# DTUWindEnergy/WindGym

Hardware: AMD Instinct MI355X
Metric: env-steps/sec (whole node), 16-turbine farm x 4096 envs (higher is better)
Workload: dtype f32

## Files before the change

### windgym_amd/csrc/wg_env.hip

```cpp
#include <hip/hip_runtime.h>

#ifndef WG_ENV_ABLATE
#define WG_ENV_ABLATE 0
#endif
#include "wg_env_common.h"
#include "wg_internal.h"

struct __attribute__((aligned(16))) EnvSlotLds {
    int dev_rem, fill_rem, sub, budget;
    double s_new;
    int n_emit, n_valid, new_valid;
    unsigned n_emitted;
    float s_off_f, near_f, move_max, ti_pow;
    double s_off, ws;
    float ws_f, ti_f, wd_env, base_acc;
    int n_pushed, pend_farm_n, pend_base_n, n_flow;
    double c_time;
    int c_head;
    unsigned c_part, c_flow, c_istep, c_tag, n_emitted0;
    float out_pw;
    unsigned c_add;
    int bg_init;
    int pad_[3];
};
// ... 133 lines not shown
            c_tag = (unsigned)cx.episode_tag; init_pending = cx.init_pending; time_max_c = cx.time_max;
            const int* ro = kl->d.roff + ctx_id * (unsigned)(N + 1);
            l_roff = ro[(unsigned)t]; l_rnext = ro[(unsigned)t + 1u];
            l_xr = kl->d.xr[tcx]; l_yr = kl->d.yr[tcx];
            l_yaw = kl->d.yaw[tb]; l_u = kl->d.u[tb]; l_ti = kl->d.ti_loc[tb];
            l_bnd = reinterpret_cast<const float4*>(kl->d.bnd)[tb];
        };
        load_state();
        const int n_tab = k0->p.n_tab, S = k0->p.S;
        const unsigned i_tab = (unsigned)min(tid, n_tab - 1), i_s = (unsigned)min(tid, S - 1);
        const float pf_tp = k0->d.tab_power[i_tab], pf_tc = k0->d.tab_ct[i_tab];
        const float pf_dy = k0->d.rotor_dy[i_s], pf_dz = k0->d.rotor_dz[i_s];
        {
            const bool has_act = mode == WG_MODE_STEP && farm == 0;
            const float a = *(has_act ? actions + (unsigned)(e * N + t) : k0->d.tab_ct);
            l_act = has_act ? a : 0.f;
        }

#define WG_HDR_I(f) __builtin_amdgcn_readlane(hw, (int)(offsetof(WgEnv, f) / 4))
        env_live = WG_HDR_I(live);
        int env_done = WG_HDR_I(done), env_shadow_iters = WG_HDR_I(shadow_iters), env_steps_done = WG_HDR_I(steps_done);
        int env_timestep = WG_HDR_I(timestep), env_time_max_live = WG_HDR_I(time_max_live);
#undef WG_HDR_I
        if (SPLIT && role == 1) {
            if (tid == 0) { *reinterpret_cast<int*>(smem + WG_ENV_OFF_HDR) = 0; if (GLUE != 0 && (SPLIT == 1 || wv == 0)) reinterpret_cast<int*>(zone)[LEAN_PRE_FLAG] = 0; }
            asm volatile("s_waitcnt vmcnt(0) lgkmcnt(0)" ::: "memory");
        }
        if (WPE == 2) {
            asm volatile("" : "+s"(env_live), "+s"(env_done), "+s"(env_shadow_iters), "+s"(env_steps_done), "+s"(env_timestep), "+s"(env_time_max_live) : : "memory");
            asm volatile("s_barrier" ::: "memory");
        }
        if (SPLIT && role == 1 && GLUE != 0 && c == env_live) {
            const EnvKArgsPtr kz = (EnvKArgsPtr)wg_cold_args();
            const WgParams& zp = *(const WgParams*)&kz->gp;
            const WgPtrs& zd = *(const WgPtrs*)&kz->gd;
#define WG_HDR_Z(f) __builtin_amdgcn_readlane(hw, (int)(offsetof(WgEnv, f) / 4))
            const int z_np = WG_HDR_Z(n_pushed_live), z_fn = WG_HDR_Z(farm_pow_n), z_bn = WG_HDR_Z(base_pow_n);
#undef WG_HDR_Z
            const int PA = zp.power_avg;
            const SumsRaw zr = wg_sums_load<false, false>(zp, zd, e, e * 2 + env_live, tid < N ? tid : 0, z_np);
            const float z_fo = zd.farm_pow[(size_t)e * PA + z_fn % PA];
            const float z_bo = F == 2 ? zd.base_pow[(size_t)e * PA + z_bn % PA] : 0.f;
            const float z_met = tid < WG_N_METRICS ? zd.metrics[(size_t)e * WG_N_METRICS + tid] : 0.f;
            double* const zs = reinterpret_cast<double*>(zone);
#pragma unroll
            for (int sI = 0; sI < WG_N_CH; ++sI) { zs[LEAN_PRE_S(sI, tid)] = zr.S[sI]; zone[LEAN_PRE_LV(sI, tid)] = zr.lv[sI]; }
            zone[LEAN_PRE_MET(tid)] = z_met;
            if (tid == 0) { zone[LEAN_PRE_FOLD] = z_fo; zone[LEAN_PRE_BOLD] = z_bo; }
            asm volatile("s_waitcnt lgkmcnt(0)" ::: "memory");
            if (tid == 0) env_flag_set(reinterpret_cast<int*>(zone) + LEAN_PRE_FLAG);
        }
        out.env_live = env_live;
        out.truncates = env_timestep >= env_time_max_live;
        out.steps_done = env_steps_done; out.time_max_live = env_time_max_live;

        const bool is_live_c = (c == env_live);
        const int autoreset = k0->p.autoreset;
        int budget = 0;
        long plan_left = 0;
        if (mode == WG_MODE_STEP) {
            role_live = is_live_c && !env_done;
            role_dev = !is_live_c && autoreset != 0;
            const int bg_pending = WPE == 2 ? (is_live_c ? 0 : __shfl(init_pending, 0, 64)) : __shfl(init_pending, (env_live ^ 1) * F * N, 64);
            out.bg_init_pending = autoreset && bg_pending;
            if (SPLIT == 2 && role == 1 && out.bg_init_pending) return;
            if (autoreset && bg_pending && WPE == 1 && !out.truncates) {
                defer_init = true;
                budget = 0;
            } else if (autoreset && bg_pending) {
                const KArgsPtr ki = wg_cold_args();
                const WgParams& gp = *ki->d.gp;
                env_init_episode<GLUE != 0>(e, env_live ^ 1, tid);
                full_barrier<64>();
                load_state();
                const int fill_max = F == 2 ? max(gp.fill_a, gp.fill_b) : gp.fill_a;
                const int inc = 1 + (gp.extra_inc ? 1 : 0);
                const int tm = WPE == 2 ? ki->d.ctx[e * 2 + env_live].time_max : __shfl(time_max_c, env_live * F * N, 64);
                const long total = (long)((tm + inc - 1) / inc) + 1;
                const int dev0 = __shfl(dev_rem, WPE == 2 ? 0 : (env_live ^ 1) * F * N, 64);
                budget = wg_shadow_share(dev0 + gp.K * fill_max, total - env_steps_done, env_steps_done, e);
                budget = wg_shadow_share(dev_rem + gp.K * fill_rem, total - env_steps_done, env_steps_done, e, farm ? 0x80000000u : 0u);
// ... 68 lines not shown
        float2* const rpt = reinterpret_cast<float2*>(tabct + n_tab);
        const float hub = k1->p.hub;
        auto rp = [&](const float dy_, const float dz_) __attribute__((always_inline)) {
            const float dz = hub + dz_ - hub;
            return make_float2(dy_, dz * dz);
        };
        if (tid < n_tab) { tabp[tid] = pf_tp; tabct[tid] = pf_tc; }
        if (tid < S) rpt[tid] = rp(pf_dy, pf_dz);
        for (int i = tid + 64; i < n_tab; i += 64) { tabp[i] = k1->d.tab_power[i]; tabct[i] = k1->d.tab_ct[i]; }
        for (int i = tid + 64; i < S; i += 64) rpt[i] = rp(k1->d.rotor_dy[i], k1->d.rotor_dz[i]);

        yaw = l_yaw; tu = l_u; tti = l_ti; oyaw = l_yaw;
        if (role_live && farm == 0 && valid) {
            const float a = l_act, ymin = k1->p.yaw_min, ymax = k1->p.yaw_max, ystep = k1->p.yaw_step;
            if (k1->p.action_method == WG_ACT_YAW) {
                yaw = fminf(fmaxf(yaw + a * ystep, ymin), ymax);
            } else {
                float tf = a + 1.0f;
                tf = tf * 0.5f;
                tf = tf * (ymax - ymin);
                tf = tf + ymin;
                const float ny = fminf(fmaxf(tf, yaw - ystep), yaw + ystep);
                yaw = fminf(fmaxf(ny, ymin), ymax);
            }
        }
    }
    float tpow = 0.f, tct = 0.f, cg = 1.f;
    float sws = 0.f, swd = 0.f, syaw = 0.f, sp_ = 0.f;
    int part_acc = 0, stream_acc = 0;
    bool stepped = false;
    lds_barrier<64>();
    WG_STAMP(1);

    for (int round = 0;; ++round) {
        bool stepping, is_dev;
        int sub, K;
        if (__ballot(parked)) {
            bool due = parked && SL[k - 1].dev_rem == 0;
            unsigned long long due_m = __ballot(due);
            if (due_m) {
                full_barrier<64>();
                const KArgsPtr kc = wg_cold_args();
                const unsigned pstride = (unsigned)kc->p.pstride;
                const size_t pb_env = (size_t)(e * 2 * F + kbase) * pstride;
                const int src_lane = (tid - N) & 63;
                const float c_tu = __shfl(tu, src_lane, 64), c_tti = __shfl(tti, src_lane, 64), c_pw = __shfl(tpow, src_lane, 64);
                const float c_ct = __shfl(tct, src_lane, 64), c_cg = __shfl(cg, src_lane, 64);
                if (due) { tu = c_tu; tti = c_tti; tpow = c_pw; tct = c_ct; cg = c_cg; stepped = true; parked = false; }
                while (due_m) {
                    const int kd = __builtin_amdgcn_readlane(k, __builtin_ctzll(due_m));
                    env_clone_dev(smem, kd, N, kc->p.P, kc->p.dt_d, kc->d.py + pb_env, kc->d.rec_a + 2 * pb_env, (unsigned)(kd - 1) * pstride,
                                  (unsigned)kd * pstride, tid);
                    due_m &= ~(((1ull << N) - 1ull) << (kd * N));
                }
                lds_barrier<64>();
            }
        }
        {
            const KArgsPtr kr = wg_cold_args();
            K = kr->p.K;
            const int4 sch = *reinterpret_cast<const int4*>(&my.dev_rem);
            const bool active = sch.x > 0 || sch.y > 0;
            stepping = valid && (role_live ? (round < K) : (role_dev && active && (sch.w > 0 || sch.z != 0)));
            is_dev = !role_live && sch.x > 0;
            sub = sch.z;
            if (!__ballot(stepping)) break;
        out.rounds = round + 1;
            if (round > 0) full_barrier<64>();

            if (role_live && farm == 1 && stepping) {
                const float ystep = kr->p.yaw_step;
                if (kr->p.base_controller == WG_CTRL_LOCAL) {
                    const float off = 0.f - yaw;
                    const float sgn = (float)((off > 0.f) - (off < 0.f));
                    yaw = yaw + sgn * fminf(fabsf(off), ystep);
                } else {
                    const float sgn = (float)((yaw > 0.f) - (yaw < 0.f));
                    yaw = yaw - sgn * fminf(fabsf(yaw), ystep);
                }
            }

            if (stepping && t == 0) {
                const double dpart = kr->p.dpart;
                const int P = kr->p.P;
                const double s_off = my.s_off, adv = my.ws * kr->p.dt_d;
                double s_new = s_off + adv;
                int n_emit = 0;
                while (s_new >= dpart) { s_new -= dpart; ++n_emit; }
// ... 321 lines not shown
                            pyv[i] = y0; rav[i] = rn.x; rbv[i] = rn.y;
                        }
                    }
                    reinterpret_cast<uint4*>(ra_env)[2u * q] = make_uint4(rav[0], rbv[0], rav[1], rbv[1]);
                    reinterpret_cast<uint4*>(ra_env)[2u * q + 1u] = make_uint4(rav[2], rbv[2], rav[3], rbv[3]);
                }
                reinterpret_cast<float4*>(py_env)[q] = make_float4(pyv[0], pyv[1], pyv[2], pyv[3]);
                float ex = 0.f;
#pragma unroll
                for (int i = 0; i < 4; ++i) {
                    int j = j0 - i; if (j < 0) j += R;
                    if (j < n_valid_q) ex = fmaxf(ex, fabsf(pyv[i] - y0));
                }
                if (ex > Lsrc2[gq].x) atomicMax(reinterpret_cast<int*>(&Lsrc2[gq].x), __float_as_int(ex));
            };
            QuadReq qa, qb;
            qa.py = qb.py = make_float4(0.f, 0.f, 0.f, 0.f); qa.ra = qa.rb = qb.ra = qb.rb = make_uint4(0u, 0u, 0u, 0u);
            request(qa, tid);
            if (SPLIT && role == 1) {
                if (!env_flag_wait(reinterpret_cast<int*>(smem + WG_ENV_OFF_HDR))) atomicOr(kp->d.status, WG_STATUS_BIT_STATE);
            }
            for (int base = 0; base < nlist; base += 64) {
                qb = qa;
                request(qa, base + 64 + tid);
                advect_quad(qb, base + tid);
            }
        }
        lds_barrier<64>();
        WG_STAMP(3);
        if (SPLIT && role == 1) {
            if (stepping) reinterpret_cast<float4*>(wg_cold_args()->d.bnd)[(unsigned)((e * 2 * F + kbase) * N + g)].x = Lsrc2[g].x;
            return;
        }

        const bool measuring = stepping && !is_dev;
        const bool unit_end = measuring && (sub + 1 == K);
        const KArgsPtr kc = wg_cold_args();
        const float inv_k = 1.0f / (float)K;
        const unsigned ctx_id = (unsigned)(e * 2 + c);
        if (stepping) {
            {
                int4 rg = Lring[g];
                const int n_emit = my.n_emit;
                rg.z += n_emit;
                if (n_emit >= rg.y) rg.z %= rg.y; else if (rg.z >= rg.y) rg.z -= rg.y;
                Lring[g].z = rg.z;
                part_acc += min(my.new_valid, rg.y);
            }
            stepped = true;
            const int n_tab = kc->p.n_tab;
            const float tab_x0 = kc->p.tab_x0, tab_inv_dx = kc->p.tab_inv_dx;
            const float* const tabp = reinterpret_cast<const float*>(smem + kc->p.env_off_tab);
            const float wsn = fmaxf(tu * cg, 0.0f);
            tpow = env_tab(tabp, tab_x0, tab_inv_dx, n_tab, wsn);
            tct = env_tab(tabp + n_tab, tab_x0, tab_inv_dx, n_tab, wsn) * cg * cg;
            if (measuring && farm == 0) {
                const float wsm = __builtin_amdgcn_sqrtf(tu * tu);
                const float wdm = 0.f + my.wd_env;
                float val[WG_N_CH] = {sws + wsm, swd + wdm, syaw + yaw, sp_ + tpow};
                if (unit_end) {
                    const int n_pushed = my.n_pushed;
                    const unsigned tcx = ctx_id * (unsigned)N + (unsigned)t;
                    kc->d.cur_ws[tcx] = wsm;
                    kc->d.cur_wd[tcx] = wdm;
                    if (K != 1) {
#pragma unroll
// ... 93 lines not shown
            const double dt_d = ke->p.dt_d;
            double tm = my.c_time;
            for (int i = 0; i < n_flow; ++i) tm += dt_d;
            const unsigned n_emitted = my.n_emitted;
            int hd = my.c_head + (int)((n_emitted - my.n_emitted0) % (unsigned)P); if (hd >= P) hd -= P;
            WgSlot& slot = ke->d.slot[(unsigned)(e * 2 * F + kbase + k)];
            slot.part_count = my.c_part + (unsigned)part_slot;
            slot.add_count = my.c_add + (unsigned)stream_slot;
            slot.head = hd; slot.n_valid = my.n_valid; slot.s_off = my.s_off; slot.time = tm;
            slot.istep = my.c_istep + (unsigned)n_flow; slot.n_emitted = n_emitted;
            slot.dev_remaining = my.dev_rem; slot.fill_remaining = my.fill_rem;
            slot.flow_count = my.c_flow + (unsigned)n_flow;
            WgCtx& cx = ke->d.ctx[(unsigned)(e * 2 + c)];
            if (farm == 0) { cx.n_pushed = my.n_pushed; cx.pend_farm_n = my.pend_farm_n; }
            if (farm == F - 1) cx.pend_base_n = my.pend_base_n;
        }
    }
    if (GLUE != 0) {
        out.g_yaw = yaw; out.g_old = oyaw; out.g_pw = tpow;
        out.g_pwb = F == 2 ? __shfl(tpow, min(tid + N, 63), 64) : 0.f;
    }
    WG_STAMP(8);
    if (mode == WG_MODE_STEP && (WPE == 1 || c != env_live) && !defer_init) {
        const EnvSlotLds& bs = SL[WPE == 2 ? 0 : (env_live ^ 1) * F];
        const int bctx = e * 2 + (env_live ^ 1);
        bool build = false;
        if (ke->p.autoreset && bs.dev_rem == 0 && bs.fill_rem == 0)
            build = bs.n_flow == 0 ? (ke->d.gd->next_obs_ok != nullptr && ke->d.gd->next_obs_ok[bctx] == 0) : out.truncates != 0;
        if (build) {
            const int np = bs.n_pushed;
            out.first_obs = 1;
            full_barrier<64>();
            env_first_obs<GLUE != 0>(bctx, np, tid);
        }
    }
    if (defer_init) {
        env_init_episode<GLUE != 0>(e, env_live ^ 1, tid);
        full_barrier<64>();
        if (valid && t == 0 && c != env_live) {
            const WgSlot& slot = ke->d.slot[(unsigned)(e * 2 * F + kbase + k)];
            my.dev_rem = slot.dev_remaining; my.fill_rem = slot.fill_remaining;
        }
        lds_barrier<64>();
    }
}


template <bool NOISE, int GLUE, int WPE, int SPLIT = 0>
__global__ void __launch_bounds__(64 * (WPE + SPLIT), WG_ENV_WAVES)
k_flow_env(const FlowP p_, const FlowPtrs d_, const int mode, const float* __restrict__ actions,
           const uint8_t* __restrict__ mask, const int chunk, const WgParams gp_, const WgPtrs gd_,
           float* __restrict__ obs_out, float* __restrict__ reward_out, uint8_t* __restrict__ trunc_out,
           float* __restrict__ final_obs_out) {
    extern __shared__ __attribute__((aligned(16))) char smem[];
#ifdef WG_TIMELINE
    if (threadIdx.x == 0) { for (int i = 0; i < 20; ++i) wg_stamps[i] = 0; wg_stamps[14] = wall_clock64(); for (int i = 0; i < 8; ++i) wg_counts[i] = 0; }
    __syncthreads();
#endif
    const int wv4 = WPE == 2 ? __builtin_amdgcn_readfirstlane((int)(threadIdx.x >> 6)) : 0;
    int wv = wv4, role = 0;
    if (SPLIT == 1 && wv4 == 2) {
        role = 1;
        wv = __builtin_amdgcn_readfirstlane(reinterpret_cast<const int*>(wg_cold_args()->d.env + blockIdx.x)[offsetof(WgEnv, live) / 4]) & 1;
    }
    if (SPLIT == 2) { wv = wv4 & 1; role = wv4 >> 1; }
    const int lds_wave = WPE == 2 ? wg_cold_args()->p.env_lds : 0;
    char* const sm = smem + wv4 * lds_wave;
    char* const sm_pass = smem + (SPLIT == 2 ? 2 + wv : 2) * lds_wave;
    float* const zone = SPLIT ? reinterpret_cast<float*>(smem + (2 + SPLIT) * lds_wave) : nullptr;
    EnvFlowOut fo;
    env_flow<NOISE, WPE, GLUE, SPLIT>(sm, sm_pass, zone, wv, role, mode, actions, mask, chunk, fo);
    if (SPLIT && role == 1) {
        if (GLUE != 0 && fo.truncates) { __builtin_amdgcn_s_waitcnt(0x0070); __syncthreads(); }
        return;
    }
    if (GLUE != 0) {
        if (SPLIT != 0 || fo.truncates) full_barrier<64>();
        if (WPE == 2) {
            if (wv != fo.env_live) {
                const EnvKArgsPtr kb = (EnvKArgsPtr)wg_cold_args();
                const int e = (int)blockIdx.x;
                if (kb->p.autoreset && !fo.truncates && (threadIdx.x & 63) == 0) {
                    const int F = kb->p.F, K = kb->p.K;
                    const EnvSlotLds* const SLb = reinterpret_cast<const EnvSlotLds*>(sm + WG_ENV_OFF_SL);
                    int work = 0;
                    for (int f = 0; f < F; ++f) work = max(work, SLb[f].dev_rem + K * SLb[f].fill_rem);
                    env_bg_plan(kb, work, fo, e);
                }
                if (fo.bg_init_pending && (threadIdx.x & 63) == 0) kb->d.ctx[e * 2 + wv].init_pending = 0;
                if (fo.truncates) __builtin_amdgcn_s_waitcnt(0x0070);
            }
            if (fo.truncates) __syncthreads();
        }
        if (WPE == 1 || wv == fo.env_live) {
            const EnvKArgsPtr kg = (EnvKArgsPtr)wg_cold_args();
            const int F = kg->p.F, K = kg->p.K;
            const EnvSlotLds* const SLa = reinterpret_cast<const EnvSlotLds*>(sm + WG_ENV_OFF_SL);
            const int la = WPE == 2 ? 0 : fo.env_live * F, lb = (fo.env_live ^ 1) * F;
            const float fp = SLa[la].out_pw, bp = F == 2 ? SLa[la + 1].out_pw : 0.f;
            int work = 0;
            if (WPE == 1) for (int f = 0; f < F; ++f) work = max(work, SLa[lb + f].dev_rem + K * SLa[lb + f].fill_rem);
            const int hw = reinterpret_cast<const int*>(sm + WG_ENV_OFF_HDR)[threadIdx.x & 31];
            LeanFused fz;
            fz.pre = nullptr; fz.regs = SPLIT == 0;
            if (SPLIT) {
                if (!env_flag_wait(reinterpret_cast<int*>(zone) + LEAN_PRE_FLAG)) atomicOr(kg->d.status, WG_STATUS_BIT_STATE);
                fz.pre = zone;
            }
            const int gl = (int)(threadIdx.x & 63), own = gl < kg->p.N ? gl : 0;
            if (WPE == 2) {
#pragma unroll
                for (int ch = 0; ch < WG_N_CH; ++ch) fz.nw[ch] = __shfl(fo.g_nw[ch], own, 64);
                fz.yaw = fo.g_yaw; fz.old_yaw = fo.g_old; fz.pw = fo.g_pw; fz.pwb = fo.g_pwb;
            } else {
                const int src = fo.env_live * F * kg->p.N + own;
#pragma unroll
                for (int ch = 0; ch < WG_N_CH; ++ch) fz.nw[ch] = __shfl(fo.g_nw[ch], src, 64);
                fz.yaw = __shfl(fo.g_yaw, src, 64); fz.old_yaw = __shfl(fo.g_old, src, 64);
                fz.pw = __shfl(fo.g_pw, src, 64); fz.pwb = __shfl(fo.g_pwb, src, 64);
            }
            WG_STAMP(12);
            env_glue<GLUE, WPE>(kg, fz, fp, bp, work, fo, hw);
            WG_STAMP(13);
        }
    }
#ifdef WG_TIMELINE
    {
        const KArgsPtr kt = wg_cold_args();
        if (threadIdx.x == 0 && kt->d.dbg) {
            wg_stamps[15] = wall_clock64();
            long long* row = kt->d.dbg + (size_t)blockIdx.x * 32;
            for (int kq = 0; kq < 16; ++kq) row[kq] = wg_stamps[kq];
            row[16] = fo.bg_init_pending; row[17] = fo.rounds; row[18] = fo.first_obs;
            row[19] = GLUE != 0 ? (long long)kt->d.env[blockIdx.x].timestep : 0;
            for (int kq = 0; kq < 8; ++kq) row[20 + kq] = wg_counts[kq];
            for (int kq = 0; kq < 4; ++kq) row[28 + kq] = wg_stamps[16 + kq];
        }
    }
#endif
}

template <bool NZ, int G>
static EnvKernel env_kernel(const int wpe, const int split) {
    if constexpr (G != 0) {
        if (split == 2) return k_flow_env<NZ, G, 2, 2>;
        if (split == 1) return k_flow_env<NZ, G, 2, 1>;
    }
    return wpe == 2 ? k_flow_env<NZ, G, 2> : k_flow_env<NZ, G, 1>;
}
static void env_launch(const FlowP* p, const FlowPtrs* d, const int glue, const int mode, const float* actions, const uint8_t* mask,
                       const int chunk, const WgParams* gp, const WgPtrs* gd, float* obs, float* reward, uint8_t* trunc,
                       float* final_obs, hipStream_t st) {
    const int wpe = p->env_wpe == 2 ? 2 : 1;
    const int split = glue != 0 && wpe == 2 && (p->env_split == 1 || p->env_split == 2) ? p->env_split : 0;
    const size_t lds = (size_t)p->env_lds * (wpe + split) + (split ? LEAN_PRE_BYTES : 0);
// ... 18 lines not shown
```

### windgym_amd/csrc/wg_env_common.h

```cpp
#pragma once
#include <hip/hip_runtime.h>

#include "wg_flow_dev.h"
#include "wg_glue_lean.h"

#ifndef WG_ENV_WAVES
#define WG_ENV_WAVES 4
#endif

static __device__ __attribute__((noinline)) void env_init_episode_mem(const WgParams* gp, const WgPtrs* gd, WgEnv* env_rw,
                                                                      const int e, const int c, const int lane) {
    const WgCtx& cx = gd->ctx[e * 2 + c];
    WgRng rng{cx.snap_state, cx.snap_inc, cx.snap_has32, cx.snap_u32};
    wg_ctx_init(*gp, *gd, rng, e, c, lane, cx.episode_tag, 0, gp->F);
    if (lane == 0) {
        env_rw->rng_state = rng.rng_state; env_rw->rng_inc = rng.rng_inc;
        env_rw->rng_has32 = rng.rng_has32; env_rw->rng_u32 = rng.rng_u32;
    }
}
struct EnvKArgs;
template <bool KARG>
__device__ __forceinline__ void env_init_episode(const int e, const int c, const int lane);

__device__ __forceinline__ float env_tab(const float* __restrict__ ys, const float x0, const float inv_dx, const int n_tab, const float x) {
// ... 85 lines not shown
#pragma unroll
                for (int u = 0; u < 8; ++u)
                    if (k + u * Lg < cnt) acc += (double)v[u];
            }
        }
        for (int s2 = 1; s2 < Lg; s2 <<= 1) acc += __shfl_xor(acc, s2, 64);
        if (on && sub == 0) ws_[(size_t)sl * NS] = acc;
        if (have && sub == 0 && n_pushed > 0) {
            if ((cmask >> sl) & 1u) o[n++] = wg_scale_r(cv[sl], p.oc.mn[sl], p.oc.inv_rng[sl]);
            if ((rmask >> sl) & 1u) o[n++] = wg_scale_r(wg_sums_mean(p.oc, acc, sl, n_pushed), p.oc.mn[sl], p.oc.inv_rng[sl]);
        }
    }
    if (lane == 0) d.next_obs_ok[ctx_id] = 1;
}

__device__ __forceinline__ void env_flag_set(int* const f) {
    __atomic_store_n(f, 1, __ATOMIC_RELAXED);
    asm volatile("s_waitcnt lgkmcnt(0)" ::: "memory");
}
__device__ __forceinline__ bool env_flag_wait(int* const f) {
    for (int n = 0; n < (1 << 22); ++n) {
        if (__atomic_load_n(f, __ATOMIC_RELAXED) != 0) { asm volatile("" ::: "memory"); return true; }
        __builtin_amdgcn_s_sleep(2);
    }
    return false;
}

struct EnvFlowOut {
    int env_live, bg_init_pending;
    int truncates;
    int steps_done, time_max_live;
    int rounds, first_obs;
    float g_nw[WG_N_CH], g_yaw, g_old, g_pw, g_pwb;
};


__device__ __forceinline__ void env_bg_plan(const EnvKArgsPtr kb, const int work, const EnvFlowOut& fo, const int e) {
    const int steps_done = fo.steps_done + 1, time_max = fo.time_max_live;
    const int inc = 1 + (kb->gp.extra_inc ? 1 : 0);
    const long total = (long)((time_max + inc - 1) / inc) + 1;
    kb->d.env_rw[e].shadow_iters = work == 0 ? 0 : wg_shadow_share(work, total - steps_done, steps_done, e);
}

template <int GLUE, int WPE>
__device__ __forceinline__ void env_glue(const EnvKArgsPtr kg, LeanFused& fz, const float fp, const float bp, const int work,
                                         const EnvFlowOut& fo, const int hw) {
    fz.fp = fp; fz.bp = bp; fz.work = work;
    fz.bg_init_pending = WPE >= 2 ? 0 : fo.bg_init_pending;
    fz.plan_elsewhere = WPE >= 2;
    fz.hw = hw;
    lean_step<GLUE == 2, false, true>(*(const WgParams*)&kg->gp, *(const WgPtrs*)&kg->gd, kg->d.gp, kg->d.gd, (int)blockIdx.x,
                                      (int)(threadIdx.x & 63), kg->obs, kg->reward, kg->trunc, kg->final_obs, nullptr, fz);
}

typedef void (*EnvKernel)(FlowP, FlowPtrs, int, const float*, const uint8_t*, int, WgParams, WgPtrs, float*, float*, uint8_t*, float*);
```

### windgym_amd/csrc/wg_envb.hip

```cpp
#include <hip/hip_runtime.h>

#include "wg_env_common.h"
#include "wg_box_dev.h"
#include "wg_internal.h"

#ifndef WG_ENVB_U
#define WG_ENVB_U 2
#endif
#ifndef WG_ENVB_ABLATE
#define WG_ENVB_ABLATE 0
#endif
#ifndef WG_ENVB_WAVES
#define WG_ENVB_WAVES 4
#endif

struct __attribute__((aligned(16))) EnvbSlotLds {
    int dev_rem, fill_rem, sub, budget;
    double s_new;
    int n_emit, n_valid, new_valid;
    unsigned n_emitted;
    float s_off_f, ti_pow, sig, alpha;
    double s_off, ws;
    float ws_f, ti_f, wd_env, base_acc;
    int n_pushed, pend_farm_n, pend_base_n, n_flow;
// ... 941 lines not shown
                    if (WPE == 4) {
                        if (!envb_flag_wait(flags + wv + 1)) atomicOr(kb->d.status, WG_STATUS_BIT_STATE);
                        for (int f = 0; f < F; ++f) {
                            const EnvbSlotLds* const s_ = reinterpret_cast<const EnvbSlotLds*>(smem + (wv + f) * lds_wave + LO::SL);
                            work = max(work, s_->dev_rem + K * s_->fill_rem);
                        }
                    } else {
                        const EnvbSlotLds* const SLb = reinterpret_cast<const EnvbSlotLds*>(sm + LO::SL);
                        for (int f = 0; f < F; ++f) work = max(work, SLb[f].dev_rem + K * SLb[f].fill_rem);
                    }
                    env_bg_plan(kb, work, fo, e);
                }
                if (fo.bg_init_pending && lane0) kb->d.ctx[e * 2 + c_w].init_pending = 0;
            }
            if (c_w != fo.env_live && fo.truncates) __builtin_amdgcn_s_waitcnt(0x0070);
            if (fo.truncates) __syncthreads();
        }
        if (WPE == 1 || (c_w == fo.env_live && farm_w == 0)) {
            const EnvKArgsPtr kg = (EnvKArgsPtr)wg_cold_args();
            float fp, bp;
            int work = 0;
            if (WPE == 4) {
                if (F == 2 && !envb_flag_wait(flags + wv + 1)) { if (lane0) atomicOr(kg->d.status, WG_STATUS_BIT_STATE); }
                fp = reinterpret_cast<const EnvbSlotLds*>(sm + LO::SL)->out_pw;
                bp = F == 2 ? reinterpret_cast<const EnvbSlotLds*>(sm + lds_wave + LO::SL)->out_pw : 0.f;
            } else {
                const EnvbSlotLds* const SLa = reinterpret_cast<const EnvbSlotLds*>(sm + LO::SL);
                const int la = WPE == 2 ? 0 : fo.env_live * F, lb = (fo.env_live ^ 1) * F;
                fp = SLa[la].out_pw;
                bp = F == 2 ? SLa[la + 1].out_pw : 0.f;
                if (WPE == 1) for (int f = 0; f < F; ++f) work = max(work, SLa[lb + f].dev_rem + K * SLa[lb + f].fill_rem);
            }
            LeanFused fz;
            fz.pre = nullptr; fz.regs = 0;
            env_glue<GLUE, WPE>(kg, fz, fp, bp, work, fo, reinterpret_cast<const int*>(sm + LO::HDR)[threadIdx.x & 31]);
        }
    }
}

template <bool NZ, int G>
static EnvKernel envb_kernel(const int wpe) {
    return wpe == 4 ? k_flow_envb<NZ, G, 4> : wpe == 2 ? k_flow_envb<NZ, G, 2> : k_flow_envb<NZ, G, 1>;
}
static void envb_launch(const FlowP* p, const FlowPtrs* d, const int glue, const int mode, const float* actions, const uint8_t* mask,
                        const int chunk, const WgParams* gp, const WgPtrs* gd, float* obs, float* reward, uint8_t* trunc,
                        float* final_obs, hipStream_t st) {
    const int wpe = p->env_wpe == 4 ? 4 : (p->env_wpe == 2 ? 2 : 1);
    const size_t lds = (size_t)p->env_lds * wpe + (wpe == 4 ? WG_ENVB_FLAG_BYTES : 0);
    const EnvKernel k = glue == 2 ? (p->noise ? envb_kernel<true, 2>(wpe) : envb_kernel<false, 2>(wpe))
                      : glue == 1 ? (p->noise ? envb_kernel<true, 1>(wpe) : envb_kernel<false, 1>(wpe))
                                  : (p->noise ? envb_kernel<true, 0>(wpe) : envb_kernel<false, 0>(wpe));
    hipLaunchKernelGGL(k, dim3(p->B), dim3(64 * wpe), lds, st, *p, *d, mode, actions, mask, chunk, *gp, *gd, obs, reward, trunc, final_obs);
}

extern "C" void wg_launch_flow_envb(const FlowP* p, const FlowPtrs* d, int mode, const float* actions, const uint8_t* mask,
                                    int chunk, hipStream_t st) {
    static const WgParams gp0{};
    static const WgPtrs gd0{};
    envb_launch(p, d, 0, mode, actions, mask, chunk, &gp0, &gd0, nullptr, nullptr, nullptr, nullptr, st);
}

extern "C" void wg_launch_step_envb(const FlowP* p, const FlowPtrs* d, const WgParams* gp, const WgPtrs* gd, const float* actions,
                                    float* obs, float* reward, uint8_t* trunc, float* final_obs, hipStream_t st) {
    envb_launch(p, d, gd->multi_out ? 2 : 1, WG_MODE_STEP, actions, nullptr, 0, gp, gd, obs, reward, trunc, final_obs, st);
}
```

### windgym_amd/csrc/wg_glue_lean.h

```cpp
#pragma once
#include <hip/hip_runtime.h>

#include "wg_device.h"
#include "wg_obs.h"

__device__ inline float deque_at(const float* dq, int n_total, int maxlen, int q) {
    const int n = n_total < maxlen ? n_total : maxlen;
    return dq[(n_total - n + q) % maxlen];
}

struct EnvHot {
    int live, timestep, episode, done, shadow_iters, farm_pow_n, base_pow_n, steps_done;
    float ep_return, ep_power_sum;
    int ep_len;
};
__device__ inline EnvHot env_load(const WgEnv& env) {
    EnvHot h;
    h.live = env.live; h.timestep = env.timestep; h.episode = env.episode; h.done = env.done;
    h.shadow_iters = env.shadow_iters; h.farm_pow_n = env.farm_pow_n; h.base_pow_n = env.base_pow_n;
    h.steps_done = env.steps_done; h.ep_return = env.ep_return; h.ep_power_sum = env.ep_power_sum; h.ep_len = env.ep_len;
    return h;
}
__device__ inline void env_writeback(WgEnv& env, const EnvHot& ev, const int lane, const bool skip_shadow = false) {
    if (lane == 0) env.live = ev.live;
// ... 197 lines not shown
    if (lane == 4) envw.base_pow_n = n2b;
    if (lane == 5) envw.time_max_live = time_max;
    if (lane == 6) envw.rated_live = rated;
    if (lane == 7) envw.fsum_run = sf;
    if (lane == 8) envw.bsum_run = sb;
    if (lane == 9) envw.n_pushed_live = nnp;
    if (lane == 10) envw.shadow_iters = 0;
    if (!obs_done && obs) {
        asm volatile("s_waitcnt vmcnt(0)" ::: "memory");
        auto ld = [&](const int ent) {
            ObsIn o;
            const SumsEnt q = wg_sums_ent(p, d, nctx, ent);
            const double* ws_ = d.wsum + (size_t)nctx * WG_N_SUMS * NS + ent;
#pragma unroll
            for (int sl = 0; sl < WG_N_SUMS; ++sl) o.S[sl] = ((q.sm >> sl) & 1u) ? __builtin_nontemporal_load(ws_ + (size_t)sl * NS) : 0.0;
#pragma unroll
            for (int ch = 0; ch < WG_N_CH; ++ch) {
                const int off = q.farm ? p.fring_off[ch] : p.ring_off[ch];
                o.cur[ch] = (nnp > 0 && ((q.cm >> ch) & 1u)) ? q.rb[off + ((nnp - 1) % p.ring_cap[ch]) * q.stride] : 0.f;
            }
            return o;
        };
        build_obs_sums<MULTI, GEN>(p, lane, obs, nullptr, om, nnp, mscr, ld(lane < N ? lane : 0), ld);
    }
}


#ifndef WG_LEAN_ABLATE
#define WG_LEAN_ABLATE 0
#endif
__device__ __forceinline__ int wg_uni(const int v) { return __builtin_amdgcn_readfirstlane(v); }
__device__ __forceinline__ float wg_uni(const float v) { return __int_as_float(__builtin_amdgcn_readfirstlane(__float_as_int(v))); }

struct LeanFused {
    float fp, bp;
    int work;
    int bg_init_pending;
    int plan_elsewhere;
    int hw;
    const float* pre;
    int regs;
    float nw[WG_N_CH], yaw, old_yaw, pw, pwb;
};
#define LEAN_PRE_S(s, lane) ((s) * 64 + (lane))
#define LEAN_PRE_LV(s, lane) (512 + (s) * 64 + (lane))
#define LEAN_PRE_MET(lane) (768 + (lane))
#define LEAN_PRE_FOLD 832
#define LEAN_PRE_BOLD 833
#define LEAN_PRE_FLAG 834

template <bool MULTI, bool GEN, bool FUSED>
__device__ __forceinline__ void lean_step(const WgParams& p, const WgPtrs& d, const WgParams* gp, const WgPtrs* gd, const int e,
                                          const int lane, float* __restrict__ obs_out, float* __restrict__ reward_out,
                                          uint8_t* __restrict__ trunc_out, float* __restrict__ final_obs_out, float* const mscr,
                                          const LeanFused& fz) {
    const int N = p.N, F = p.F, PA = p.power_avg;
    WgEnv& env = d.env[e];
    float* obs = obs_out ? obs_out + (size_t)e * p.obs_dim : nullptr;
    float* om = MULTI ? d.multi_out + (size_t)e * N * p.obs_dim_multi : nullptr;
    float* omf = (MULTI && d.multi_fin) ? d.multi_fin + (size_t)e * N * p.obs_dim_multi : nullptr;
    float* fq = d.farm_pow + (size_t)e * PA;
    float* bq = d.base_pow + (size_t)e * PA;
    const int own = lane < N ? lane : 0;

    static_assert(sizeof(WgEnv) == 128, "lean_step loads the env header as 32 words");
    const int hw = FUSED ? fz.hw : reinterpret_cast<const int*>(&env)[lane & 31];
#define WG_HDR_I(f) __builtin_amdgcn_readlane(hw, (int)(offsetof(WgEnv, f) / 4))
#define WG_HDR_F(f) __int_as_float(WG_HDR_I(f))
#define WG_HDR_D(f) __hiloint2double(__builtin_amdgcn_readlane(hw, (int)(offsetof(WgEnv, f) / 4) + 1), WG_HDR_I(f))
    if (WG_HDR_I(done)) {
        if (lane == 0) atomicOr(d.status, WG_STATUS_BIT_STATE);
        return;
    }
    EnvHot ev;
    ev.live = WG_HDR_I(live); ev.timestep = WG_HDR_I(timestep); ev.episode = WG_HDR_I(episode); ev.done = 0; ev.shadow_iters = 0;
    ev.farm_pow_n = WG_HDR_I(farm_pow_n); ev.base_pow_n = WG_HDR_I(base_pow_n); ev.steps_done = WG_HDR_I(steps_done);
    ev.ep_return = WG_HDR_F(ep_return); ev.ep_power_sum = WG_HDR_F(ep_power_sum); ev.ep_len = WG_HDR_I(ep_len);
    int time_max = WG_HDR_I(time_max_live), n_pushed_live = WG_HDR_I(n_pushed_live);
    float rated_power = WG_HDR_F(rated_live);
    double fsum_run = WG_HDR_D(fsum_run), bsum_run = WG_HDR_D(bsum_run);
#undef WG_HDR_D
#undef WG_HDR_F
#undef WG_HDR_I
    const int live = ev.live, nxt = live ^ 1;
#if defined(WG_TIMELINE) && defined(WG_STAMP2)
    if (FUSED) WG_STAMP2(16);
#endif
    const int ctx_id = e * 2 + live;
    if (WG_LEAN_ABLATE == 1) { if (lane == 0 && reward_out) reward_out[e] = (float)(fsum_run + bsum_run) + (float)(ev.timestep + ev.episode + time_max + n_pushed_live); return; }
    int nx_pfn = 0, nx_pbn = 0, nx_np = 0, nx_tmax = 0;
    float nx_rated = 0.f;
    bool nx_prep = false;
    if (ev.timestep >= time_max && p.autoreset) {
        const WgCtx& nc = d.ctx[e * 2 + nxt];
        nx_pfn = wg_uni(nc.pend_farm_n); nx_pbn = wg_uni(nc.pend_base_n); nx_np = wg_uni(nc.n_pushed); nx_tmax = wg_uni(nc.time_max);
        nx_rated = wg_uni(nc.rated_power);
        nx_prep = d.next_obs_ok != nullptr && wg_uni(d.next_obs_ok[e * 2 + nxt]) != 0;
    }
    const bool pre = FUSED && !GEN && fz.pre != nullptr;
    const bool regs = FUSED && !GEN && !pre && fz.regs != 0;
    SumsRaw raw;
    const bool have2 = !FUSED && lane + WG_WAVE < N;
    SumsRaw raw2 = {};
    const size_t tb_a = (size_t)(ctx_id * F) * N;
    float l_yaw = 0.f, l_old = 0.f, l_pow = 0.f, l_powb = 0.f;
    const float fp = FUSED ? fz.fp : wg_uni(d.step_farm_pow[e]);
    const float bp = F == 2 ? (FUSED ? fz.bp : wg_uni(d.step_base_pow[e])) : 0.f;
    const int fslot = ev.farm_pow_n % PA, bslot = ev.base_pow_n % PA;
    float* met = d.metrics + (size_t)e * WG_N_METRICS;
    float f_old, b_old, l_met;
    if (pre) {
        const double* const zs = reinterpret_cast<const double*>(fz.pre);
#pragma unroll
        for (int s = 0; s < WG_N_SUMS; ++s) { raw.S[s] = 0.0; raw.lv[s] = 0.f; }
#pragma unroll
        for (int s = 0; s < WG_N_CH; ++s) {
            if ((p.sum_mask_t >> s) & 1u) { raw.S[s] = zs[LEAN_PRE_S(s, lane)]; raw.lv[s] = fz.pre[LEAN_PRE_LV(s, lane)]; }
        }
        f_old = wg_uni(fz.pre[LEAN_PRE_FOLD]); b_old = F == 2 ? wg_uni(fz.pre[LEAN_PRE_BOLD]) : 0.f;
        l_met = lane < WG_N_METRICS ? fz.pre[LEAN_PRE_MET(lane)] : 0.f;
    } else {
        raw = regs ? wg_sums_load<GEN, false>(p, d, e, ctx_id, own, n_pushed_live) : wg_sums_load<GEN>(p, d, e, ctx_id, own, n_pushed_live);
        if (have2) raw2 = wg_sums_load<GEN>(p, d, e, ctx_id, lane + WG_WAVE, n_pushed_live);
        if (!regs && lane < N) {
            l_yaw = d.yaw[tb_a + lane]; l_old = d.old_yaw[(size_t)e * N + lane]; l_pow = d.power[tb_a + lane];
            if (F == 2) l_powb = d.power[tb_a + N + lane];
        }
        f_old = wg_uni(fq[fslot]); b_old = F == 2 ? wg_uni(bq[bslot]) : 0.f;
        l_met = lane < WG_N_METRICS ? met[lane] : 0.f;
    }
    if (pre || regs) {
        const unsigned msk = p.sum_mask_t | p.cur_mask_t;
#pragma unroll
        for (int ch = 0; ch < WG_N_CH; ++ch) raw.nw[ch] = ((msk >> ch) & 1u) ? fz.nw[ch] : 0.f;
        if (lane < N) { l_yaw = fz.yaw; l_old = fz.old_yaw; l_pow = fz.pw; if (F == 2) l_powb = fz.pwb; }
    }
    int work = 0;
    if (p.autoreset) {
        if (FUSED) {
            work = fz.work;
            if (fz.bg_init_pending && lane == 0) d.ctx[e * 2 + nxt].init_pending = 0;
        } else {
            const WgSlot* const bs = d.slot + (size_t)(e * 2 + nxt) * F;
            for (int f = 0; f < F; ++f) work = max(work, wg_uni(bs[f].dev_remaining) + p.K * wg_uni(bs[f].fill_remaining));
            if (wg_uni(d.ctx[e * 2 + nxt].init_pending) && lane == 0) d.ctx[e * 2 + nxt].init_pending = 0;
        }
    }
#if defined(WG_TIMELINE) && defined(WG_STAMP2)
    if (FUSED) { __builtin_amdgcn_s_waitcnt(0); WG_STAMP2(17); }
#endif
    if (WG_LEAN_ABLATE == 2) {
        float acc = raw.nw[0] + raw.nw[2] + raw.lv[0] + raw.lv[2] + (float)raw.S[0] + (float)raw.S[2] + l_yaw + l_old + l_pow + l_powb + fp + bp + f_old + b_old + l_met;
        if (reward_out) reward_out[e] = acc + (float)work;
// ... 148 lines not shown
```

### windgym_amd/csrc/wg_obs.h

```cpp
#pragma once
#include "wg_device.h"

#define WG_OBSV(v, mn, rng) (raw ? (v) : wg_clip1(wg_scale((v), (mn), (rng))))
template <int L>
__device__ inline float wg_group_sum(float s) {
#pragma unroll
    for (int o = 1; o < L; o <<= 1) s += __shfl_xor(s, o, 64);
    return s;
}
template <int L>
__device__ inline float wg_ring_sum_g(const WgRing& r, const int lo, const int hi, const int sub) {
    constexpr int U = L == 1 ? 8 : 4;
    float s = 0.f;
#pragma nounroll
    for (int q = lo + sub; q < hi; q += U * L) {
        float v[U];
#pragma unroll
        for (int k = 0; k < U; ++k) v[k] = r.at(min(q + k * L, hi - 1));
#pragma unroll
        for (int k = 0; k < U; ++k)
            if (q + k * L < hi) s += v[k];
    }
    return wg_group_sum<L>(s);
}
// ... 130 lines not shown
                            int spacing = (avail - W) / (HN - 1); if (spacing < 1) spacing = 1;
                            int pos = i * spacing; if (pos > avail - W) pos = avail - W;
                            lo = pos; hi = pos + W;
                        }
                        const float s = wg_ring_sum(r, lo, hi);
                        float v = WG_OBSV(s / (float)(hi - lo), p.sc_min[ch], rng);
                        o[n] = v; if (o2) o2[n] = v; ++n;
                    }
                }
            }
        }
    }
}

struct ObsIn {
    double S[WG_N_SUMS];
    float cur[WG_N_CH];
};
struct SumsRaw {
    double S[WG_N_SUMS];
    float nw[WG_N_CH];
    float lv[WG_N_SUMS];
};
__device__ __forceinline__ int wg_umod(int n, int H, unsigned magic) {
    if (H == 1) return 0;
    int r = n - (int)__umulhi((unsigned)n, magic) * H;
    if (r >= H) r -= H;
    if (r < 0) r += H;
    return r;
}
struct SumsEnt {
    const float* rb; int stride; bool farm; unsigned sm, cm;
};
__device__ __forceinline__ SumsEnt wg_sums_ent(const WgParams& p, const WgPtrs& d, const int ctx_id, const int ent) {
    SumsEnt q;
    q.farm = ent == p.N;
    q.rb = q.farm ? d.fring + (size_t)ctx_id * p.fring_stride : d.ring + (size_t)ctx_id * p.ring_stride + ent;
    q.stride = q.farm ? 1 : p.N;
    q.sm = q.farm ? p.sum_mask_f : p.sum_mask_t;
    q.cm = q.farm ? p.cur_mask_f : p.cur_mask_t;
    return q;
}
template <bool GEN, bool NEWEST = true>
__device__ inline SumsRaw wg_sums_load(const WgParams& p, const WgPtrs& d, const int e, const int ctx_id, const int ent, const int np) {
    constexpr int NSL = GEN ? WG_N_SUMS : WG_N_CH;
    SumsRaw r;
    const SumsEnt q = wg_sums_ent(p, d, ctx_id, ent);
    const int NS = p.N + 1;
    const double* ws_ = d.wsum + (size_t)ctx_id * WG_N_SUMS * NS + ent;
    const unsigned ti = GEN ? q.sm >> WG_SUM_TI1 : 0u;
#pragma unroll
    for (int ch = 0; ch < WG_N_CH; ++ch) {
        const bool need = (((q.sm | q.cm) >> ch) & 1u) || (ch == WG_CH_WS && ti);
        const int off = q.farm ? p.fring_off[ch] : p.ring_off[ch];
        r.nw[ch] = (NEWEST && need) ? q.rb[off + wg_umod(np, p.ring_cap[ch], p.ring_magic[ch]) * q.stride] : 0.f;
    }
#pragma unroll
    for (int s = 0; s < WG_N_SUMS; ++s) { r.S[s] = 0.0; r.lv[s] = 0.f; }
#pragma unroll
    for (int s = 0; s < NSL; ++s) {
        if ((q.sm >> s) & 1u) {
            const int ch = s < WG_N_CH ? s : WG_CH_WS;
            const int off = q.farm ? p.fring_off[ch] : p.ring_off[ch];
            const int Wc = p.sum_w[s];
            r.S[s] = ws_[(size_t)s * NS];
            if (np >= Wc) r.lv[s] = q.rb[off + wg_umod(np - Wc, p.ring_cap[ch], p.ring_magic[ch]) * q.stride];
        }
    }
    return r;
}
template <bool GEN>
__device__ inline ObsIn wg_sums_apply(const WgParams& p, const WgPtrs& d, const int ctx_id, const int ent, const SumsRaw& r, const bool store) {
    constexpr int NSL = GEN ? WG_N_SUMS : WG_N_CH;
    ObsIn o;
    const int NS = p.N + 1;
    const unsigned sm = ent == p.N ? p.sum_mask_f : p.sum_mask_t;
    double* ws_ = d.wsum + (size_t)ctx_id * WG_N_SUMS * NS + ent;
#pragma unroll
    for (int s = 0; s < WG_N_SUMS; ++s) o.S[s] = 0.0;
#pragma unroll
// ... 113 lines not shown
```

Baseline: 90.61 million.

## Prefetch lean glue sums and power history early in the fused non-split path

Adds a LeanEarly helper that loads the windowed sums, last-value terms, old farm/base power and metrics for the glue step. In the fused non-split path it issues these loads at earlier points in the flow loop (after clones, barriers and first-obs) so global-memory latency can overlap other work instead of stalling inside lean_step. It also specialises the sums loader for turbine-only entries and pins the lane index in a vector register. The cost is more live registers carried across the flow loop, which may reduce occupancy, plus loads repeated at several call sites.

```diff
diff --git a/windgym_amd/csrc/wg_env.hip b/windgym_amd/csrc/wg_env.hip
--- a/windgym_amd/csrc/wg_env.hip
+++ b/windgym_amd/csrc/wg_env.hip
@@ -189,21 +189,12 @@
         }
         if (SPLIT && role == 1 && GLUE != 0 && c == env_live) {
             const EnvKArgsPtr kz = (EnvKArgsPtr)wg_cold_args();
-            const WgParams& zp = *(const WgParams*)&kz->gp;
-            const WgPtrs& zd = *(const WgPtrs*)&kz->gd;
-#define WG_HDR_Z(f) __builtin_amdgcn_readlane(hw, (int)(offsetof(WgEnv, f) / 4))
-            const int z_np = WG_HDR_Z(n_pushed_live), z_fn = WG_HDR_Z(farm_pow_n), z_bn = WG_HDR_Z(base_pow_n);
-#undef WG_HDR_Z
-            const int PA = zp.power_avg;
-            const SumsRaw zr = wg_sums_load<false, false>(zp, zd, e, e * 2 + env_live, tid < N ? tid : 0, z_np);
-            const float z_fo = zd.farm_pow[(size_t)e * PA + z_fn % PA];
-            const float z_bo = F == 2 ? zd.base_pow[(size_t)e * PA + z_bn % PA] : 0.f;
-            const float z_met = tid < WG_N_METRICS ? zd.metrics[(size_t)e * WG_N_METRICS + tid] : 0.f;
+            const LeanEarly zr = lean_early_load(*(const WgParams*)&kz->gp, *(const WgPtrs*)&kz->gd, e, N, F, tid, hw);
             double* const zs = reinterpret_cast<double*>(zone);
 #pragma unroll
             for (int sI = 0; sI < WG_N_CH; ++sI) { zs[LEAN_PRE_S(sI, tid)] = zr.S[sI]; zone[LEAN_PRE_LV(sI, tid)] = zr.lv[sI]; }
-            zone[LEAN_PRE_MET(tid)] = z_met;
-            if (tid == 0) { zone[LEAN_PRE_FOLD] = z_fo; zone[LEAN_PRE_BOLD] = z_bo; }
+            zone[LEAN_PRE_MET(tid)] = zr.met;
+            if (tid == 0) { zone[LEAN_PRE_FOLD] = zr.f_old; zone[LEAN_PRE_BOLD] = zr.b_old; }
             asm volatile("s_waitcnt lgkmcnt(0)" ::: "memory");
             if (tid == 0) env_flag_set(reinterpret_cast<int*>(zone) + LEAN_PRE_FLAG);
         }
@@ -338,6 +329,17 @@
     lds_barrier<64>();
     WG_STAMP(1);
 
+    auto glue_early = [&]() __attribute__((always_inline)) {
+        if (GLUE != 0 && SPLIT == 0) {
+            if (WPE == 2 && wv != env_live) {
+                out.g_early = LeanEarly{};
+            } else {
+                const EnvKArgsPtr kz = (EnvKArgsPtr)wg_cold_args();
+                const int hwl = reinterpret_cast<const int*>(smem + WG_ENV_OFF_HDR)[tid & 31];
+                out.g_early = lean_early_load(*(const WgParams*)&kz->gp, *(const WgPtrs*)&kz->gd, e, N, F, tid, hwl);
+            }
+        }
+    };
     for (int round = 0;; ++round) {
         bool stepping, is_dev;
         int sub, K;
@@ -360,6 +362,7 @@
                     due_m &= ~(((1ull << N) - 1ull) << (kd * N));
                 }
                 lds_barrier<64>();
+                glue_early();
             }
         }
         {
@@ -747,6 +750,7 @@
             if (stepping) reinterpret_cast<float4*>(wg_cold_args()->d.bnd)[(unsigned)((e * 2 * F + kbase) * N + g)].x = Lsrc2[g].x;
             return;
         }
+        glue_early();
 
         const bool measuring = stepping && !is_dev;
         const bool unit_end = measuring && (sub + 1 == K);
@@ -906,6 +910,7 @@
             out.first_obs = 1;
             full_barrier<64>();
             env_first_obs<GLUE != 0>(bctx, np, tid);
+            glue_early();
         }
     }
     if (defer_init) {
@@ -916,6 +921,7 @@
             my.dev_rem = slot.dev_remaining; my.fill_rem = slot.fill_remaining;
         }
         lds_barrier<64>();
+        glue_early();
     }
 }
 
@@ -976,12 +982,15 @@
             if (WPE == 1) for (int f = 0; f < F; ++f) work = max(work, SLa[lb + f].dev_rem + K * SLa[lb + f].fill_rem);
             const int hw = reinterpret_cast<const int*>(sm + WG_ENV_OFF_HDR)[threadIdx.x & 31];
             LeanFused fz;
-            fz.pre = nullptr; fz.regs = SPLIT == 0;
+            fz.pre = nullptr; fz.regs = SPLIT == 0; fz.early = SPLIT == 0;
+            if (SPLIT == 0) fz.ev = fo.g_early;
             if (SPLIT) {
                 if (!env_flag_wait(reinterpret_cast<int*>(zone) + LEAN_PRE_FLAG)) atomicOr(kg->d.status, WG_STATUS_BIT_STATE);
                 fz.pre = zone;
             }
-            const int gl = (int)(threadIdx.x & 63), own = gl < kg->p.N ? gl : 0;
+            int gl = (int)(threadIdx.x & 63);
+            asm volatile("" : "+v"(gl));
+            const int own = gl < kg->p.N ? gl : 0;
             if (WPE == 2) {
 #pragma unroll
                 for (int ch = 0; ch < WG_N_CH; ++ch) fz.nw[ch] = __shfl(fo.g_nw[ch], own, 64);
@@ -994,7 +1003,7 @@
                 fz.pw = __shfl(fo.g_pw, src, 64); fz.pwb = __shfl(fo.g_pwb, src, 64);
             }
             WG_STAMP(12);
-            env_glue<GLUE, WPE>(kg, fz, fp, bp, work, fo, hw);
+            env_glue<GLUE, WPE>(kg, fz, fp, bp, work, fo, hw, gl);
             WG_STAMP(13);
         }
     }
diff --git a/windgym_amd/csrc/wg_env_common.h b/windgym_amd/csrc/wg_env_common.h
--- a/windgym_amd/csrc/wg_env_common.h
+++ b/windgym_amd/csrc/wg_env_common.h
@@ -141,6 +141,7 @@
     int steps_done, time_max_live;
     int rounds, first_obs;
     float g_nw[WG_N_CH], g_yaw, g_old, g_pw, g_pwb;
+    LeanEarly g_early;
 };
 
 
@@ -153,13 +154,13 @@
 
 template <int GLUE, int WPE>
 __device__ __forceinline__ void env_glue(const EnvKArgsPtr kg, LeanFused& fz, const float fp, const float bp, const int work,
-                                         const EnvFlowOut& fo, const int hw) {
+                                         const EnvFlowOut& fo, const int hw, const int lane = (int)(threadIdx.x & 63)) {
     fz.fp = fp; fz.bp = bp; fz.work = work;
     fz.bg_init_pending = WPE >= 2 ? 0 : fo.bg_init_pending;
     fz.plan_elsewhere = WPE >= 2;
     fz.hw = hw;
     lean_step<GLUE == 2, false, true>(*(const WgParams*)&kg->gp, *(const WgPtrs*)&kg->gd, kg->d.gp, kg->d.gd, (int)blockIdx.x,
-                                      (int)(threadIdx.x & 63), kg->obs, kg->reward, kg->trunc, kg->final_obs, nullptr, fz);
+                                      lane, kg->obs, kg->reward, kg->trunc, kg->final_obs, nullptr, fz);
 }
 
 typedef void (*EnvKernel)(FlowP, FlowPtrs, int, const float*, const uint8_t*, int, WgParams, WgPtrs, float*, float*, uint8_t*, float*);
diff --git a/windgym_amd/csrc/wg_envb.hip b/windgym_amd/csrc/wg_envb.hip
--- a/windgym_amd/csrc/wg_envb.hip
+++ b/windgym_amd/csrc/wg_envb.hip
@@ -997,7 +997,7 @@
                 if (WPE == 1) for (int f = 0; f < F; ++f) work = max(work, SLa[lb + f].dev_rem + K * SLa[lb + f].fill_rem);
             }
             LeanFused fz;
-            fz.pre = nullptr; fz.regs = 0;
+            fz.pre = nullptr; fz.regs = 0; fz.early = 0;
             env_glue<GLUE, WPE>(kg, fz, fp, bp, work, fo, reinterpret_cast<const int*>(sm + LO::HDR)[threadIdx.x & 31]);
         }
     }
diff --git a/windgym_amd/csrc/wg_glue_lean.h b/windgym_amd/csrc/wg_glue_lean.h
--- a/windgym_amd/csrc/wg_glue_lean.h
+++ b/windgym_amd/csrc/wg_glue_lean.h
@@ -253,6 +253,26 @@
 __device__ __forceinline__ int wg_uni(const int v) { return __builtin_amdgcn_readfirstlane(v); }
 __device__ __forceinline__ float wg_uni(const float v) { return __int_as_float(__builtin_amdgcn_readfirstlane(__float_as_int(v))); }
 
+struct LeanEarly {
+    double S[WG_N_CH];
+    float lv[WG_N_CH], f_old, b_old, met;
+};
+__device__ __forceinline__ LeanEarly lean_early_load(const WgParams& p, const WgPtrs& d, const int e, const int N, const int F,
+                                                     const int lane, const int hw) {
+#define WG_HDR_Z(f) __builtin_amdgcn_readlane(hw, (int)(offsetof(WgEnv, f) / 4))
+    const int z_live = WG_HDR_Z(live), z_np = WG_HDR_Z(n_pushed_live), z_fn = WG_HDR_Z(farm_pow_n), z_bn = WG_HDR_Z(base_pow_n);
+#undef WG_HDR_Z
+    const int PA = p.power_avg;
+    const SumsRaw zr = wg_sums_load<false, false, true>(p, d, e, e * 2 + z_live, lane < N ? lane : 0, z_np);
+    LeanEarly q;
+#pragma unroll
+    for (int s = 0; s < WG_N_CH; ++s) { q.S[s] = zr.S[s]; q.lv[s] = zr.lv[s]; }
+    q.f_old = d.farm_pow[(size_t)e * PA + z_fn % PA];
+    q.b_old = F == 2 ? d.base_pow[(size_t)e * PA + z_bn % PA] : 0.f;
+    q.met = lane < WG_N_METRICS ? d.metrics[(size_t)e * WG_N_METRICS + lane] : 0.f;
+    return q;
+}
+
 struct LeanFused {
     float fp, bp;
     int work;
@@ -262,6 +282,8 @@
     const float* pre;
     int regs;
     float nw[WG_N_CH], yaw, old_yaw, pw, pwb;
+    int early;
+    LeanEarly ev;
 };
 #define LEAN_PRE_S(s, lane) ((s) * 64 + (lane))
 #define LEAN_PRE_LV(s, lane) (512 + (s) * 64 + (lane))
@@ -320,6 +342,7 @@
     }
     const bool pre = FUSED && !GEN && fz.pre != nullptr;
     const bool regs = FUSED && !GEN && !pre && fz.regs != 0;
+    const bool early = regs && fz.early != 0;
     SumsRaw raw;
     const bool have2 = !FUSED && lane + WG_WAVE < N;
     SumsRaw raw2 = {};
@@ -340,6 +363,13 @@
         }
         f_old = wg_uni(fz.pre[LEAN_PRE_FOLD]); b_old = F == 2 ? wg_uni(fz.pre[LEAN_PRE_BOLD]) : 0.f;
         l_met = lane < WG_N_METRICS ? fz.pre[LEAN_PRE_MET(lane)] : 0.f;
+    } else if (early) {
+#pragma unroll
+        for (int s = 0; s < WG_N_SUMS; ++s) { raw.S[s] = 0.0; raw.lv[s] = 0.f; }
+#pragma unroll
+        for (int s = 0; s < WG_N_CH; ++s) { raw.S[s] = fz.ev.S[s]; raw.lv[s] = fz.ev.lv[s]; }
+        f_old = wg_uni(fz.ev.f_old); b_old = F == 2 ? wg_uni(fz.ev.b_old) : 0.f;
+        l_met = fz.ev.met;
     } else {
         raw = regs ? wg_sums_load<GEN, false>(p, d, e, ctx_id, own, n_pushed_live) : wg_sums_load<GEN>(p, d, e, ctx_id, own, n_pushed_live);
         if (have2) raw2 = wg_sums_load<GEN>(p, d, e, ctx_id, lane + WG_WAVE, n_pushed_live);
diff --git a/windgym_amd/csrc/wg_obs.h b/windgym_amd/csrc/wg_obs.h
--- a/windgym_amd/csrc/wg_obs.h
+++ b/windgym_amd/csrc/wg_obs.h
@@ -186,20 +186,21 @@
 struct SumsEnt {
     const float* rb; int stride; bool farm; unsigned sm, cm;
 };
+template <bool TURB = false>
 __device__ __forceinline__ SumsEnt wg_sums_ent(const WgParams& p, const WgPtrs& d, const int ctx_id, const int ent) {
     SumsEnt q;
-    q.farm = ent == p.N;
+    q.farm = TURB ? false : ent == p.N;
     q.rb = q.farm ? d.fring + (size_t)ctx_id * p.fring_stride : d.ring + (size_t)ctx_id * p.ring_stride + ent;
     q.stride = q.farm ? 1 : p.N;
     q.sm = q.farm ? p.sum_mask_f : p.sum_mask_t;
     q.cm = q.farm ? p.cur_mask_f : p.cur_mask_t;
     return q;
 }
-template <bool GEN, bool NEWEST = true>
+template <bool GEN, bool NEWEST = true, bool TURB = false>
 __device__ inline SumsRaw wg_sums_load(const WgParams& p, const WgPtrs& d, const int e, const int ctx_id, const int ent, const int np) {
     constexpr int NSL = GEN ? WG_N_SUMS : WG_N_CH;
     SumsRaw r;
-    const SumsEnt q = wg_sums_ent(p, d, ctx_id, ent);
+    const SumsEnt q = wg_sums_ent<TURB>(p, d, ctx_id, ent);
     const int NS = p.N + 1;
     const double* ws_ = d.wsum + (size_t)ctx_id * WG_N_SUMS * NS + ent;
     const unsigned ti = GEN ? q.sm >> WG_SUM_TI1 : 0u;
```

New measurement: 92.14 million (median of 6 runs). 1.02x the previous value.
